# lixinghe1999/VRVQ

Hardware: AMD Instinct MI355X
Metric: audio-sec/s encode+RVQ+decode, 44.1 kHz batch-32, 1->8 MI355X; RVQ HBM GB/s (higher is better)
Workload: dtype f32; 1 GPU; DAC_VRVQ VBR 8 cb, level 1.0, 1-s clips, preprocess+encode+decode (z_q_is materialised); model=DAC_VRVQ base (8 cb), global_batch=32, clip_samples=44100, n_codebooks=8, parallelism=dp1 (replicas, no data-path collective)

## Files before the change

### include/vrvq.h

```cpp
#ifndef VRVQ_H_
#define VRVQ_H_

#include <stdint.h>

#ifdef __cplusplus
extern "C" {
#endif

typedef void* vrvq_stream_t;

enum vrvq_status_t {
  VRVQ_OK = 0,
  VRVQ_ERR_ARG = 10001,
  VRVQ_ERR_UNSUPPORTED = 10002
};

enum vrvq_epilogue_t { VRVQ_EPI_NONE = 0, VRVQ_EPI_TANH = 1, VRVQ_EPI_SIGMOID = 2 };

const char* vrvq_status_string(int status);
int vrvq_version(void);


int vrvq_weight_norm(const float* g, const float* v, int rows, int cols, float* w,
                     vrvq_stream_t stream);

int vrvq_snake_inv_alpha(const float* alpha, int channels, float* inv, vrvq_stream_t stream);

int vrvq_snake(const float* x, int batch, int channels, int frames, const float* alpha,
               const float* inv_alpha, float* y, vrvq_stream_t stream);

int vrvq_phase_split(const float* x, int batch, int channels, int frames, int stride, int pad,
                     int out_frames, const float* alpha, const float* inv_alpha, float* y,
                     vrvq_stream_t stream);

int vrvq_codebook_prep(const float* cb, int rows, int dim, float* cbn, float* c2,
                       vrvq_stream_t stream);

int vrvq_conv1d(const float* x, int batch, int cin, int tin, const float* alpha,
                const float* inv_alpha, const float* w_packed, const uint16_t* w_x3, int cout,
                int cout_pad, int k,
                int stride, int pad, int dil, const float* bias, const float* residual,
                int epilogue, float* y, int tout, const float* alpha_out,
                const float* inv_alpha_out, float* y_snake, vrvq_stream_t stream);

int vrvq_conv1d_workspace(int batch, int cin, int tin, int cout, int k, int stride, int pad,
                          int dil, int x3, long long* bytes);
int vrvq_conv1d_ws(const float* x, int batch, int cin, int tin, const float* alpha,
                   const float* inv_alpha, const float* w_packed, const uint16_t* w_x3, int cout,
                   int cout_pad, int k, int stride, int pad, int dil, const float* bias,
                   const float* residual, int epilogue, float* y, int tout,
                   const float* alpha_out, const float* inv_alpha_out, float* y_snake,
                   void* workspace, long long ws_bytes, vrvq_stream_t stream);

int vrvq_x3_weight_size(int cin, int k, int cout_pad, long long* n_u16);
int vrvq_pack_x3_weight(const float* w_packed, int cin, int k, int cout_pad, uint16_t* w_x3,
                        vrvq_stream_t stream);

int vrvq_conv1d_proj(const float* x, int batch, int cin, int tin, const float* alpha,
                     const float* inv_alpha, const float* w_packed, const uint16_t* w_x3, int cout,
                     int cout_pad, int k, int pad, int dil, const float* bias, float* y, int tout,
                     const uint16_t* w3in, int nq, float* part, void* workspace,
                     long long ws_bytes, vrvq_stream_t stream);

int vrvq_conv_last_launch(int out[5]);

enum vrvq_plan_kind_t { VRVQ_PLAN_CONV = 0, VRVQ_PLAN_PROJ = 1, VRVQ_PLAN_CONV_TRANSPOSE = 2 };
int vrvq_conv_plan(int kind, int batch, int cin, int tin, int cout, int k, int stride, int pad,
                   int dil, int has_x3, int has_workspace, int out[7]);

int vrvq_pack_conv1d_weight(const float* w, int cout, int cin, int k, int cout_pad,
                            float* w_packed, vrvq_stream_t stream);

int vrvq_residual_unit(const float* x, const float* x_snk, int batch, int channels, int frames,
                       int dil, const float* w7_packed, const uint16_t* w7_x3,
                       const uint16_t* w1_x3, const float* b7,
                       const float* alpha2,
                       const float* inv_alpha2, const float* w1_packed, const float* b1,
                       int cout_pad, float* y, const float* alpha_out,
                       const float* inv_alpha_out, float* y_snake, vrvq_stream_t stream);

int vrvq_conv_transpose1d(const float* x, int batch, int cin, int tin, const float* alpha,
                          const float* inv_alpha, const float* w_packed, int cout,
                          int cout_pad, int stride, const float* bias, float* y,
                          const float* alpha_out, const float* inv_alpha_out, float* y_snake,
                          vrvq_stream_t stream);

int vrvq_conv_transpose1d_pad(const float* x, int batch, int cin, int tin, const float* alpha,
                              const float* inv_alpha, const float* w_packed,
                              const uint16_t* w_x3, int cout,
                              int cout_pad, int stride, int pad, const float* bias, float* y,
                              const float* alpha_out, const float* inv_alpha_out,
                              float* y_snake, vrvq_stream_t stream);

int vrvq_pack_convt1d_weight(const float* w, int cin, int cout, int stride, int cout_pad,
                             float* w_packed, vrvq_stream_t stream);


int vrvq_rvq_cross_prep(const float* w_in_t, const float* w_out, const float* b_out, int nq,
                        int dim, int cdim, float* mcol, float* qb, vrvq_stream_t stream);

int vrvq_rvq_frag(const float* cbn, int nq, int ncode, int cdim, float* cbf,
                  vrvq_stream_t stream);

int vrvq_rvq_project_variant(int variant);

int vrvq_rvq_workspace(int batch, int frames, int nq, long long* bytes);

int vrvq_rvq_path(int path);

int vrvq_rvq_sync_error(vrvq_stream_t stream, int* code);
int vrvq_rvq_pending_error(int* code);
int vrvq_rvq_debug(unsigned spin_max, unsigned stall);

int vrvq_rvq_timing(int on);
int vrvq_rvq_timing_read(float* mean_ms, int* count);

int vrvq_rvq_w_in_planes_size(int nq, int dim, int cdim, long long* n_u16);
int vrvq_rvq_pack_w_in(const float* w_in_t, int nq, int dim, int cdim, uint16_t* w3in,
                       vrvq_stream_t stream);

int vrvq_rvq_workspace_part(int batch, int frames, int nq, int ncode, long long* bytes);
// ... 146 lines not shown
```

### vrvq_amd/_lib.py

```python
from __future__ import annotations

import ctypes
import os
import threading

LIB_NAME = "libvrvq_hip.so"
LIB_PATH = os.environ.get("VRVQ_LIB") or os.path.join(os.path.dirname(os.path.abspath(__file__)), LIB_NAME)

_P = ctypes.c_void_p
_I = ctypes.c_int
_F = ctypes.c_float

SIGNATURES = {
    "vrvq_weight_norm": [_P, _P, _I, _I, _P, _P],
    "vrvq_snake_inv_alpha": [_P, _I, _P, _P],
    "vrvq_snake": [_P, _I, _I, _I, _P, _P, _P, _P],
    "vrvq_phase_split": [_P, _I, _I, _I, _I, _I, _I, _P, _P, _P, _P],
    "vrvq_codebook_prep": [_P, _I, _I, _P, _P, _P],
    "vrvq_conv1d": [_P, _I, _I, _I, _P, _P, _P, _P, _I, _I, _I, _I, _I, _I, _P, _P, _I, _P, _I,
                    _P, _P, _P, _P],
    "vrvq_conv1d_workspace": [_I, _I, _I, _I, _I, _I, _I, _I, _I, _P],
    "vrvq_conv1d_ws": [_P, _I, _I, _I, _P, _P, _P, _P, _I, _I, _I, _I, _I, _I, _P, _P, _I, _P,
                       _I, _P, _P, _P, _P, ctypes.c_longlong, _P],
    "vrvq_conv1d_proj": [_P, _I, _I, _I, _P, _P, _P, _P, _I, _I, _I, _I, _I, _P, _P, _I, _P, _I,
# ... 16 lines not shown
    "vrvq_rvq_pack_w_in": [_P, _I, _I, _I, _P, _P],
    "vrvq_rvq_workspace_part": [_I, _I, _I, _I, _P],
    "vrvq_rvq_encode_part": [_P, _I, _I, _I, _I, _I, _I, _P, _P, _P, _P, _P, _P, _P, _P, _P, _F,
                             _P, _P, _P, _P, _P, _P, _P, ctypes.c_longlong, _P],
    "vrvq_rvq_fused_clips": [_I, _I, _I, _P],
    "vrvq_rvq_project": [_P, _I, _I, _I, _I, _I, _P, _P, _P],
    "vrvq_rvq_chain": [_P, _I, _I, _I, _I, _I, _P, _P, _P, _P, _P, _P, _P, _F, _P, _P, _P, _P, _P,
                       _P],
    "vrvq_rvq_expand": [_P, _I, _I, _I, _I, _I, _P, _P, _P, _F, _P, _P, _P, _P],
    "vrvq_rvq_gather": [_P, _I, _I, _I, _P, _I, _I, _P, _P, _P, _P],
    "vrvq_masked_loss": [_P, _P, _I, _I, _I, _P, _P],
    "vrvq_mask_hard": [_P, _I, _I, _I, _P, _P],
    "vrvq_scale_imp": [_P, _I, _F, _F, _P, _P],
    "vrvq_masked_sum": [_P, _P, _I, _I, _I, _I, _P, _P],
    "vrvq_bpf": [_P, _P, _I, _I, _I, _P, _P],
    "vrvq_rate_curve": [_P, _I, _I, _I, _P, _P, _I, _P, _P],
    "vrvq_rate_solve": [_P, _I, _I, _I, _P, _P, _I, _P, _F, _F, _P, _P, _P, _P],
    "vrvq_scale_imp_rows": [_P, _I, _I, _P, _P, _P],
    "vrvq_signal_metrics_workspace": [_I, ctypes.c_longlong, _P],
    "vrvq_signal_metrics": [_P, _P, _I, _I, ctypes.c_longlong, _P, _P, _P, _P, ctypes.c_longlong,
                            _P],
    "vrvq_spectral_distance_workspace": [_I, ctypes.c_longlong, _I, _P, _P],
    "vrvq_spectral_distance": [_P, _P, _I, _I, ctypes.c_longlong, _P, _I, _P, _P, _P, _P, _P,
                               ctypes.c_double, ctypes.c_double, ctypes.c_double, ctypes.c_double,
                               _P, _P, _P, ctypes.c_longlong, _P],
    "vrvq_pack_counts": [_P, _I, _I, _I, _P, _P, _P, _P, _P],
    "vrvq_pack_codes": [_P, _P, _P, _I, _I, _I, _I, _P, _P, _P],
    "vrvq_unpack_offsets": [_P, _I, _I, _P, _P, _P],
    "vrvq_unpack_codes": [_P, _P, _P, _I, _I, _I, _P, _P, _P],
    "vrvq_rvq_nearest": [_P, _I, _I, _I, _I, _P, _P, _I, _I, _P, _P],
    "vrvq_wgrad_plan": [_I, _I, _I, _I, _I, _P, _P],
    "vrvq_conv1d_wgrad": [_P, _I, _I, _I, _P, _P, _P, _I, _I, _P, _P, _I, _I, _I, _I, _I, _P,
                          ctypes.c_longlong, _P, _P],
    "vrvq_snake_backward_workspace": [_I, _I, _I, _P],
    "vrvq_snake_backward": [_P, _P, _P, _P, _I, _I, _I, _P, _P, _P, ctypes.c_longlong, _P],
    "vrvq_bias_grad_workspace": [_I, _I, _I, _P],
    "vrvq_bias_grad": [_P, _I, _I, _I, _P, _P, ctypes.c_longlong, _P],
    "vrvq_act_backward": [_P, _P, ctypes.c_longlong, _I, _P, _P],
    "vrvq_weight_norm_backward": [_P, _P, _P, _I, _I, _P, _P, _P],
    "vrvq_pack_conv1d_flip": [_P, _I, _I, _I, _I, _P, _P],
    "vrvq_mask_ste": [_P, _P, _P, _I, _I, _I, _F, _I, _I, _P, _P],
    "vrvq_mask_ste_backward": [_P, _P, _P, _I, _I, _I, _F, _I, _P, _P],
    "vrvq_rvq_expand_masked": [_P, _I, _I, _I, _I, _I, _P, _P, _P, _P, _P, _P],
    "vrvq_rvq_backward_workspace": [_I, _I, _I, _P],
    "vrvq_rvq_backward": [_P, _P, _P, _P, _P, _P, _P, _P, _I, _I, _I, _I, _I, _I, _P, _P, _P,
                          _P, _P, _P, _P, _P, _P, _P, _P, _P, _P, ctypes.c_longlong, _P],
}
EXTRA = {"vrvq_status_string": ([_I], ctypes.c_char_p), "vrvq_version": ([], _I),
         "vrvq_rvq_project_variant": ([_I], _I), "vrvq_rvq_path": ([_I], _I),
         "vrvq_rvq_sync_error": ([_P, _P], _I), "vrvq_rvq_timing": ([_I], _I),
         "vrvq_rvq_timing_read": ([_P, _P], _I), "vrvq_rvq_pending_error": ([_P], _I),
         "vrvq_rvq_debug": ([ctypes.c_uint, ctypes.c_uint], _I),
         "vrvq_rvq_debug_capacity": ([_I], _I), "vrvq_conv_last_launch": ([_P], _I),
         "vrvq_conv_plan": ([_I] * 11 + [_P], _I)}

METRICS_CHUNK = 16384
SPECTRAL_TILE_SAMPLES = 8192


def spectral_tile_frames(window: int) -> int:
    return SPECTRAL_TILE_SAMPLES // int(window)

_lock = threading.Lock()
_lib = None


def load() -> ctypes.CDLL:
    global _lib
    if _lib is not None:
        return _lib
    with _lock:
        if _lib is not None:
            return _lib
        if not os.path.exists(LIB_PATH):
            raise RuntimeError(
                f"vrvq_amd: HIP library {LIB_PATH} is missing; build it with "
                "`python -c 'import __graft_entry__ as g; g.build()'` (hipcc, gfx950)")
        lib = ctypes.CDLL(LIB_PATH)
        for name, argtypes in SIGNATURES.items():
            fn = getattr(lib, name)
            fn.argtypes = argtypes
            fn.restype = _I
        for name, (argtypes, restype) in EXTRA.items():
            fn = getattr(lib, name)
            fn.argtypes = argtypes
            fn.restype = restype
        _lib = lib
    return _lib


def call(name: str, *args) -> None:
    lib = load()
    rc = getattr(lib, name)(*args)
    if rc != 0:
        msg = lib.vrvq_status_string(rc)
        raise RuntimeError(f"{name} failed ({rc}): {msg.decode() if msg else 'unknown'}")


def rvq_path(path: int = 0) -> int:
    prev = load().vrvq_rvq_path(path)
    if prev not in (1, 2):
        raise RuntimeError(f"vrvq_rvq_path({path}) failed ({prev})")
    return prev


def rvq_sync_error(stream: int) -> int:
    code = ctypes.c_int(0)
    call("vrvq_rvq_sync_error", ctypes.c_void_p(stream), ctypes.byref(code))
    return code.value


def rvq_pending_error() -> int:
    code = ctypes.c_int(0)
    call("vrvq_rvq_pending_error", ctypes.byref(code))
    return code.value


def rvq_debug(spin_max: int = 0, stall: int = 0) -> None:
    call("vrvq_rvq_debug", ctypes.c_uint(spin_max), ctypes.c_uint(stall))


def rvq_fused_clips(frames: int, nq: int, ncode: int = 1024) -> int:
    n = ctypes.c_int(0)
    call("vrvq_rvq_fused_clips", frames, nq, ncode, ctypes.byref(n))
    return n.value


def rvq_debug_capacity(clips: int) -> int:
    return int(load().vrvq_rvq_debug_capacity(int(clips)))


def conv_last_launch() -> dict:
    out = (ctypes.c_int * 5)()
    call("vrvq_conv_last_launch", out)
    return dict(zip(("BM", "BN", "KS", "x3", "S"), (int(v) for v in out)))


PLAN_KINDS = {"conv": 0, "proj": 1, "convt": 2}


def conv_plan(kind, batch: int, cin: int, tin: int, cout: int, k: int, stride: int = 1,
              pad: int = 0, dil: int = 1, x3: bool = True, workspace: bool = True) -> dict:
    out = (ctypes.c_int * 7)()
    call("vrvq_conv_plan", PLAN_KINDS.get(kind, kind), batch, cin, tin, cout, k, stride, pad, dil,
         1 if x3 else 0, 1 if workspace else 0, out)
    return dict(zip(("BM", "BN", "KS", "x3", "S", "path", "WM"), (int(v) for v in out)))


def rvq_timing(on: bool) -> bool:
    return bool(load().vrvq_rvq_timing(1 if on else 0))


def rvq_timing_read():
    ms, n = ctypes.c_float(0.0), ctypes.c_int(0)
    call("vrvq_rvq_timing_read", ctypes.byref(ms), ctypes.byref(n))
    return float(ms.value), int(n.value)


def rvq_project_variant(variant: int = 0) -> int:
    prev = load().vrvq_rvq_project_variant(variant)
    if prev not in (1, 2, 3):
        raise RuntimeError(f"vrvq_rvq_project_variant({variant}) failed ({prev})")
    return prev
```

### vrvq_amd/csrc/conv.hip

```cpp
#include "common.h"
#include "conv_core.h"
#include "conv_x3.h"
#include <atomic>

namespace {

using namespace vrvq_conv;

template <int BM, int BN, int WM, int NW, int KS, bool X3, bool PH = false,
          bool PAIR = x3_pair<KS, BM, BN>(), bool SPLIT = false>
__global__ __launch_bounds__(64 * NW)
__attribute__((amdgpu_waves_per_eu(X3 && x3_stages<BM, BN>() == 1 ? 2 : 1)))
void conv_mfma_kernel(ConvArgs a) {
  using TC = TileCfg<BM, BN, WM, NW>;
  extern __shared__ __attribute__((aligned(16))) float smem[];
  int bid = blockIdx.x;
  int ks = 0;
  if (SPLIT) {
    ks = bid % a.ks_split;
    bid /= a.ks_split;
  }
  const int mt = bid % a.n_mt;
  bid /= a.n_mt;
  const int nt = bid % a.n_nt;
  const int b = bid / a.n_nt;
  const int m0 = mt * BM;
  const int n0 = nt * BN;
  f32x16 acc[TC::RM][TC::RN];
#pragma unroll
  for (int i = 0; i < TC::RM; ++i)
#pragma unroll
    for (int j = 0; j < TC::RN; ++j)
#pragma unroll
      for (int r = 0; r < 16; ++r) acc[i][j][r] = 0.0f;
  constexpr bool XPF = X3 && KS == 7 && PAIR && !SPLIT;
#ifdef VRVQ_X3_SB_ALL
  constexpr bool SB = true;
#else
  constexpr bool SB = KS == 1 || (KS == 2 && BN == 128) || XPF;
#endif
  if constexpr (X3) {
    if constexpr (SPLIT) {
      constexpr int CK = X3Cfg<KS, PAIR>::CK;
      const int nch = (a.cin + CK - 1) / CK, per = (nch + a.ks_split - 1) / a.ks_split;
      if (ks * per < nch)
        conv_mainloop_x3<BM, BN, WM, NW, KS, PH, PAIR, SB>(a, smem, acc, b, m0, n0, ks * per,
                                                            min(nch, (ks + 1) * per));
      constexpr int NR = TC::RM * TC::RN * 16;
      const size_t tile = ((size_t)b * a.n_nt + nt) * a.n_mt + mt;
      const size_t ntile = (size_t)gridDim.x / a.ks_split;
      float* dst = a.ks_part + ((size_t)ks * ntile + tile) * (size_t)NR * 64 * NW +
                   (threadIdx.x >> 6) * NR * 64 + (threadIdx.x & 63);
#pragma unroll
      for (int i = 0; i < TC::RM; ++i)
#pragma unroll
        for (int j = 0; j < TC::RN; ++j)
#pragma unroll
          for (int r = 0; r < 16; ++r) dst[((i * TC::RN + j) * 16 + r) * 64] = acc[i][j][r];
      return;
    }
    conv_mainloop_x3<BM, BN, WM, NW, KS, PH, PAIR, SB, XPF>(a, smem, acc, b, m0, n0);
  } else {
    conv_mainloop<BM, BN, WM, NW, KS>(a, smem, acc, b, m0, n0);
  }
  conv_epilogue<BM, BN, WM, NW>(a, smem, acc, b, m0, n0);
}

template <int BM, int BN, int WM, int NW>
__global__ __launch_bounds__(64 * NW) void conv_splitk_epilogue_kernel(ConvArgs a) {
  using TC = TileCfg<BM, BN, WM, NW>;
  extern __shared__ __attribute__((aligned(16))) float smem[];
  int bid = blockIdx.x;
  const int mt = bid % a.n_mt;
  bid /= a.n_mt;
  const int nt = bid % a.n_nt;
  const int b = bid / a.n_nt;
  constexpr int NR = TC::RM * TC::RN * 16;
  const size_t tile = blockIdx.x;
  const size_t pstride = (size_t)gridDim.x * NR * 64 * NW;
  const float* src = a.ks_part + tile * (size_t)NR * 64 * NW + (threadIdx.x >> 6) * NR * 64 +
                     (threadIdx.x & 63);
  f32x16 acc[TC::RM][TC::RN];
#pragma unroll
  for (int i = 0; i < TC::RM; ++i)
#pragma unroll
    for (int j = 0; j < TC::RN; ++j)
#pragma unroll
      for (int r = 0; r < 16; ++r) acc[i][j][r] = src[((i * TC::RN + j) * 16 + r) * 64];
  for (int s = 1; s < a.ks_split; ++s)
#pragma unroll
    for (int i = 0; i < TC::RM; ++i)
#pragma unroll
      for (int j = 0; j < TC::RN; ++j)
#pragma unroll
        for (int r = 0; r < 16; ++r)
          acc[i][j][r] = acc[i][j][r] + src[s * pstride + ((i * TC::RN + j) * 16 + r) * 64];
  conv_epilogue<BM, BN, WM, NW>(a, smem, acc, b, mt * BM, nt * BN);
}

constexpr int SMALL_BT = 256;
constexpr int SMALL_SC = 16;
constexpr int SMALL_COUT = 8;
constexpr int SMALL_WMAX = 2048;

template <int COUT>
__global__ __launch_bounds__(256) void conv_small_cout_kernel(ConvArgs a, int ks) {
  extern __shared__ __attribute__((aligned(16))) float sm[];
  float* w_s = sm;
  float* xs = sm + SMALL_WMAX;
  const int XW = SMALL_BT + (ks - 1) * a.dil;
  const int n_t = (a.ng + SMALL_BT - 1) / SMALL_BT;
  const int b = blockIdx.x / n_t;
  const int t0 = (blockIdx.x - b * n_t) * SMALL_BT;
  const int tid = threadIdx.x;
  const float* xb = a.x + (size_t)b * a.cin * a.tin;
  for (int e = tid; e < a.cin * ks * COUT; e += 256) {
    const int c = e % COUT, rk = e / COUT;
    w_s[e] = a.w[(size_t)rk * a.m_pad + c];
  }
  float acc[COUT];
#pragma unroll
  for (int c = 0; c < COUT; ++c) acc[c] = 0.0f;

  const int pmax = min(XW, a.ng - t0 + (ks - 1) * a.dil);
  for (int ci0 = 0; ci0 < a.cin; ci0 += SMALL_SC) {
    const int nc = min(SMALL_SC, a.cin - ci0);
    const int total = nc * pmax;
    for (int e0 = tid; e0 < total; e0 += 8 * 256) {
      float v[8];
#pragma unroll
      for (int u = 0; u < 8; ++u) {
// ... 163 lines not shown
    }
    const float bb = a.bias ? a.bias[co] : 0.0f;
    const size_t o = ((size_t)b * a.cout + co) * a.ylen + t0;
#pragma unroll
    for (int u = 0; u < CI1_T; ++u) v[u] = v[u] + bb;
    if (a.res) {
#pragma unroll
      for (int u = 0; u < CI1_T; ++u)
        if (full || t0 + u < a.ng) v[u] = a.res[o + u] + v[u];
    }
#pragma unroll
    for (int u = 0; u < CI1_T; ++u) v[u] = apply_epi(v[u], a.epi);
    if (a.y) {
      if (full) *reinterpret_cast<float4*>(a.y + o) = make_float4(v[0], v[1], v[2], v[3]);
      else
        for (int u = 0; u < CI1_T; ++u)
          if (t0 + u < a.ng) a.y[o + u] = v[u];
    }
    if (a.ys) {
      snake_n1<CI1_T>(v, a.alpha_o[co], a.inv_alpha_o[co]);
      if (full) *reinterpret_cast<float4*>(a.ys + o) = make_float4(v[0], v[1], v[2], v[3]);
      else
        for (int u = 0; u < CI1_T; ++u)
          if (t0 + u < a.ng) a.ys[o + u] = v[u];
    }
  }
}

enum ConvPath { PATH_MFMA = 0, PATH_SMALL_COUT = 1, PATH_CIN1 = 2 };
struct ConvPlan {
  int path;
  int BM, BN, WM;
  int KS;
  int x3;
  int S;
};

std::atomic<unsigned> g_last_launch{0};

void note_launch(const ConvPlan& p) {
  g_last_launch.store((unsigned)p.BM | (unsigned)p.BN << 9 | (unsigned)p.KS << 18 |
                      (unsigned)p.x3 << 23 | (unsigned)(p.S & 127) << 25,
                      std::memory_order_relaxed);
}

int finish(int rc, const ConvPlan& p, ConvPlan* plan) {
  if (rc == 0) {
    if (plan) *plan = p;
    else note_launch(p);
  }
  return rc;
}

int launch_kernel(void (*kernel)(ConvArgs), long long nblk, int threads, size_t lds,
                  hipStream_t st, const ConvArgs& a, bool dry) {
  if (dry) return 0;
  if (lds > 64 * 1024) {
    hipError_t e = hipFuncSetAttribute(reinterpret_cast<const void*>(kernel),
                                       hipFuncAttributeMaxDynamicSharedMemorySize, (int)lds);
    if (e != hipSuccess) return (int)e;
  }
  ConvArgs arg = a;
  void* params[] = {&arg};
  hipError_t e = hipLaunchKernel(reinterpret_cast<const void*>(kernel), dim3((unsigned)nblk),
                                 dim3(threads), params, lds, st);
  return e != hipSuccess ? (int)e : vrvq_launch_status();
}

int launch_small(const ConvArgs& a, int batch, int ks, hipStream_t st, ConvPlan* plan) {
  const ConvPlan p{PATH_SMALL_COUT, 0, 0, 0, ks, 0, 0};
  if (a.M == 1 && a.cout == 1 && a.stride == 1 && a.dil == 1 && a.tin % 4 == 0 &&
      ((ks == 7 && a.pad == 3) || (ks == 3 && a.pad == 1))) {
    const long long nblk = (long long)batch * ((a.ng + 256 * C1_T - 1) / (256 * C1_T));
    if (nblk <= 0 || nblk > 0x7fffffffLL) return VRVQ_ERR_ARG;
    if (plan) *plan = p;
    void (*kernel)(ConvArgs) =
        ks == 7 ? (a.alpha ? conv_cout1_stream_kernel<7, 3, true> : conv_cout1_stream_kernel<7, 3, false>)
                : (a.alpha ? conv_cout1_stream_kernel<3, 1, true> : conv_cout1_stream_kernel<3, 1, false>);
    return launch_kernel(kernel, nblk, 256, 0, st, a, plan != nullptr);
  }
  if (a.cin * ks * (a.M == 1 ? 1 : SMALL_COUT) > SMALL_WMAX) return VRVQ_ERR_UNSUPPORTED;
  const size_t lds = (size_t)(SMALL_WMAX + SMALL_SC * (SMALL_BT + (ks - 1) * a.dil)) * sizeof(float);
  if (lds > 64 * 1024) return VRVQ_ERR_UNSUPPORTED;
  const long long nblk = (long long)batch * ((a.ng + SMALL_BT - 1) / SMALL_BT);
  if (nblk <= 0 || nblk > 0x7fffffffLL) return VRVQ_ERR_ARG;
  if (plan) {
    *plan = p;
    return 0;
  }
  if (a.M == 1)
    hipLaunchKernelGGL(conv_small_cout_kernel<1>, dim3((unsigned)nblk), dim3(256), lds, st, a, ks);
  else
    hipLaunchKernelGGL(conv_small_cout_kernel<SMALL_COUT>, dim3((unsigned)nblk), dim3(256), lds, st, a, ks);
  return vrvq_launch_status();
}

template <int BM, int BN, int WM, int NW, int KS, bool PAIR, bool SPLIT = false>
int launch_x3(const ConvArgs& a, int XW, size_t epi, long long nblk, hipStream_t st, bool dry) {
  size_t lx = x3_lds_bytes<KS, BM, BN, PAIR>(XW, a.alpha ? (a.psh ? a.cin >> a.psh : a.cin) : 0);
  if (lx < epi) lx = epi;
  if (lx > 160 * 1024) return VRVQ_ERR_UNSUPPORTED;
  constexpr bool PH_TILE = KS == 2 && (x3_pair<KS, BM, BN>() || SPLIT);
  if constexpr (PH_TILE) {
    if (a.psh)
      return launch_kernel(conv_mfma_kernel<BM, BN, WM, NW, KS, true, true, PAIR, SPLIT>, nblk,
                           64 * NW, lx, st, a, dry);
  }
  if constexpr (SPLIT && KS == 2) {
    return VRVQ_ERR_ARG;
  } else {
    if (a.psh) return VRVQ_ERR_ARG;
    return launch_kernel(conv_mfma_kernel<BM, BN, WM, NW, KS, true, false, PAIR, SPLIT>, nblk,
                         64 * NW, lx, st, a, dry);
  }
}

template <int BM, int BN, int WM, int NW, int KS>
int launch_cfg(const ConvArgs& a0, int batch, hipStream_t st, ConvPlan* plan) {
  ConvArgs a = a0;
  a.n_mt = (a.M + BM - 1) / BM;
  a.n_nt = (a.ng + BN - 1) / BN;
  if (a.m_pad < a.n_mt * BM) return VRVQ_ERR_ARG;
  if (a.up > 0 && BM % a.up != 0) return VRVQ_ERR_UNSUPPORTED;
  constexpr int CK = ChunkCfg<KS, BM, BN>::CK;
  const int XW = (BN - 1) * a.stride + (KS - 1) * a.dil + 1;
  const int XP = a.ssh ? (XW + a.stride - 1) >> a.ssh : XW;
  const int XWP = a.ssh ? ((XP << a.ssh) + 3) & ~3 : (XW + 3) & ~3;
  size_t epi = (size_t)BM * EpiCfg<BM, BN, NW / WM>::BNP * sizeof(float);
  if (a.pj_part) {
    if (BM != 128) return VRVQ_ERR_UNSUPPORTED;
    if (epi < (size_t)PJE_LDS) epi = PJE_LDS;
  }
  const long long nblk = (long long)a.n_mt * a.n_nt * batch;
  if (nblk <= 0 || nblk > 0x7fffffffLL) return VRVQ_ERR_ARG;
  ConvPlan p{PATH_MFMA, BM, BN, WM, KS, 0, 0};
  const bool dry = plan != nullptr;
  if constexpr (NW == 4 && BM <= 192 && (KS == 1 || KS == 2 || KS == 3 || KS == 7)) {
    constexpr int XW_MAX = (BN - 1) + (KS - 1) * (KS == 7 ? 9 : 1) + 1;
    if (a.w3 != nullptr && a.stride == 1 && a.ssh == 0 && XW <= XW_MAX) {
      int rc;
      if (x3_pair<KS, BM, BN>() && a.cin % X3Cfg<KS, true>::CK == 0) {
        p.x3 = 2;
        rc = launch_x3<BM, BN, WM, NW, KS, x3_pair<KS, BM, BN>()>(a, XW, epi, nblk, st, dry);
      } else {
        p.x3 = 1;
        rc = launch_x3<BM, BN, WM, NW, KS, false>(a, XW, epi, nblk, st, dry);
      }
      if (rc != VRVQ_ERR_UNSUPPORTED) return finish(rc, p, plan);
      p.x3 = 0;
    }
  }
  if (a.psh) return VRVQ_ERR_UNSUPPORTED;
  if (XW > 64 * WinCfg<KS, BN>::PER_ROW) return VRVQ_ERR_UNSUPPORTED;
  size_t lds = 2 * (size_t)(CK * KS * BM + CK * XWP) * sizeof(float);
  if (lds < epi) lds = epi;
  if (lds > 160 * 1024) return VRVQ_ERR_UNSUPPORTED;
  return finish(launch_kernel(conv_mfma_kernel<BM, BN, WM, NW, KS, false>, nblk, 64 * NW, lds, st,
                              a, dry), p, plan);
}

constexpr int SPLITK_PARTS = 4;
constexpr int SPLITK_MIN_CHUNKS = 8;

int splitk_parts(int M, int cin, int ng, int ks, bool psh, bool up, bool x3) {
  if (!x3 || up || ng > 96 || M % 128 != 0) return 0;
  if (!(ks == 3 || ks == 7 || (ks == 2 && psh))) return 0;
  const int ck = ks == 2 ? X3Cfg<2, true>::CK : ks == 3 ? X3Cfg<3>::CK : X3Cfg<7>::CK;
  if (ks == 2 && cin % ck != 0) return 0;
  const int nch = (cin + ck - 1) / ck;
  const int S = nch / SPLITK_MIN_CHUNKS < SPLITK_PARTS ? nch / SPLITK_MIN_CHUNKS : SPLITK_PARTS;
  return S >= 2 ? S : 0;
}

size_t splitk_bytes(int S, int M, int ng, int batch) {
  return S ? (size_t)S * batch * (M / 128) * ((ng + 95) / 96) * 128 * 96 * sizeof(float) : 0;
}

template <int KS>
int launch_splitk(const ConvArgs& a0, int batch, int S, hipStream_t st, ConvPlan* plan) {
  if constexpr (KS == 2 || KS == 3 || KS == 7) {
    ConvArgs a = a0;
    a.ks_split = S;
    a.n_mt = a.M / 128;
    a.n_nt = (a.ng + 95) / 96;
    if (a.m_pad < a.n_mt * 128) return VRVQ_ERR_ARG;
    const int XW = 95 + (KS - 1) * a.dil + 1;
    constexpr int XW_MAX = 95 + (KS - 1) * (KS == 7 ? 9 : 1) + 1;
    if (XW > XW_MAX) return VRVQ_ERR_UNSUPPORTED;
    size_t epi = (size_t)128 * EpiCfg<128, 96, 1>::BNP * sizeof(float);
    if (a.pj_part && epi < (size_t)PJE_LDS) epi = PJE_LDS;
    const long long tiles = (long long)a.n_mt * a.n_nt * batch;
    if (tiles * S > 0x7fffffffLL) return VRVQ_ERR_ARG;
    const ConvPlan p{PATH_MFMA, 128, 96, 4, KS, KS == 2 ? 2 : 1, S};
    const bool dry = plan != nullptr;
    int rc = launch_x3<128, 96, 4, 4, KS, KS == 2, true>(a, XW, epi, tiles * S, st, dry);
    if (rc == 0)
      rc = launch_kernel(conv_splitk_epilogue_kernel<128, 96, 4, 4>, tiles, 256, epi, st, a, dry);
    return finish(rc, p, plan);
  } else {
    (void)a0; (void)batch; (void)S; (void)st; (void)plan;
    return VRVQ_ERR_UNSUPPORTED;
  }
}

constexpr long long BN96_MIN_WORKGROUPS = 384;

template <int KS>
int tile_width(const ConvArgs& a, int batch) {
  const bool x3_2tap = KS == 2 && a.w3 != nullptr;
  if (a.ng <= 32) return 32;
  if (a.ng <= 96) {
    if (x3_2tap) return a.up > 0 ? 96 : 32;
    return (long long)((a.M + 127) / 128) * batch >= BN96_MIN_WORKGROUPS ? 96 : 32;
  }
  auto waste = [&](int bn) { return ((a.ng + bn - 1) / bn) * bn - a.ng; };
  if (a.ng < 4096 && KS != 16 && waste(64) * 10 < waste(128) * 7 &&
      !(x3_2tap && (a.psh > 0 || a.up > 0)))
    return 64;
  return 128;
}

constexpr int K7_PAIR_MIN_COLUMNS = 640;

template <int BM, int WM, int KS>
int launch_bn(int bn, const ConvArgs& a, int batch, hipStream_t st, ConvPlan* plan) {
  if constexpr (KS != 16) {
    if (bn == 64) return launch_cfg<BM, 64, WM, 4, KS>(a, batch, st, plan);
  }
  return launch_cfg<BM, 128, WM, 4, KS>(a, batch, st, plan);
}

template <int KS>
int dispatch_tiles(const ConvArgs& a, int batch, hipStream_t st, ConvPlan* plan) {
  if (a.ks_part != nullptr) {
    const int S = splitk_parts(a.M, a.cin, a.ng, KS, a.psh > 0, a.up > 0, a.w3 != nullptr);
    if (S > 0) {
      const int rc = launch_splitk<KS>(a, batch, S, st, plan);
      if (rc != VRVQ_ERR_UNSUPPORTED) return rc;
    }
  }
  const int bn = tile_width<KS>(a, batch);
  const bool x3 = a.w3 != nullptr;
  if constexpr (KS == 2) {
    if (a.up > 0 && 128 % a.up != 0) return launch_bn<192, 2, KS>(bn <= 96 ? 64 : bn, a, batch, st, plan);
  }
  if (a.M <= 32) return launch_cfg<32, 128, 1, 4, KS>(a, batch, st, plan);
// ... 124 lines not shown
  const long long n = x3_size_u16(cin, k, cout_pad);
  if (n < 0) return VRVQ_ERR_UNSUPPORTED;
  const size_t total = (size_t)n / 8;
  const unsigned grid = (unsigned)((total + 255) / 256 < 65536 ? (total + 255) / 256 : 65536);
  u32x4* out = reinterpret_cast<u32x4*>(w_x3);
  hipStream_t st = as_stream(stream);
  switch (k) {
    case 1: hipLaunchKernelGGL(pack_x3_kernel<1>, dim3(grid), dim3(256), 0, st, w_packed, cin, cout_pad, out, total); break;
    case 2: hipLaunchKernelGGL(pack_x3_kernel<2>, dim3(grid), dim3(256), 0, st, w_packed, cin, cout_pad, out, total); break;
    case 3: hipLaunchKernelGGL(pack_x3_kernel<3>, dim3(grid), dim3(256), 0, st, w_packed, cin, cout_pad, out, total); break;
    default: hipLaunchKernelGGL(pack_x3_kernel<7>, dim3(grid), dim3(256), 0, st, w_packed, cin, cout_pad, out, total); break;
  }
  return vrvq_launch_status();
}

extern "C" int vrvq_conv1d(const float* x, int batch, int cin, int tin, const float* alpha,
                           const float* inv_alpha, const float* w_packed,
                           const uint16_t* w_x3, int cout,
                           int cout_pad, int k, int stride, int pad, int dil, const float* bias,
                           const float* residual, int epilogue, float* y, int tout,
                           const float* alpha_out, const float* inv_alpha_out, float* y_snake,
                           vrvq_stream_t stream) {
  return vrvq_conv1d_ws(x, batch, cin, tin, alpha, inv_alpha, w_packed, w_x3, cout, cout_pad, k,
                        stride, pad, dil, bias, residual, epilogue, y, tout, alpha_out,
                        inv_alpha_out, y_snake, nullptr, 0, stream);
}

extern "C" int vrvq_conv1d_workspace(int batch, int cin, int tin, int cout, int k, int stride,
                                     int pad, int dil, int x3, long long* bytes) {
  VRVQ_CHECK_ARG(bytes && batch > 0 && cin > 0 && tin > 0 && cout > 0 && k > 0 && stride > 0 &&
                 dil > 0 && pad >= 0);
  const long long tout = ((long long)tin + 2LL * pad - (long long)dil * (k - 1) - 1) / stride + 1;
  VRVQ_CHECK_ARG(tout > 0);
  int S = 0;
  if (stride > 1) {
    if (x3 && k == 2 * stride && (stride & (stride - 1)) == 0 && pad < stride)
      S = splitk_parts(cout, cin * stride, (int)tout, 2, true, false, true);
  } else {
    S = splitk_parts(cout, cin, (int)tout, k, false, false, x3 != 0);
  }
  *bytes = (long long)splitk_bytes(S, cout, (int)tout, batch);
  return 0;
}

extern "C" int vrvq_conv_last_launch(int out[5]) {
  VRVQ_CHECK_ARG(out);
  const unsigned v = g_last_launch.load(std::memory_order_relaxed);
  out[0] = (int)(v & 511);
  out[1] = (int)(v >> 9 & 511);
  out[2] = (int)(v >> 18 & 31);
  out[3] = (int)(v >> 23 & 3);
  out[4] = (int)(v >> 25 & 127);
  return 0;
}

namespace {


bool conv1d_geometry_ok(int batch, int cin, int tin, int cout, int cout_pad, int k, int stride,
                        int pad, int dil, int tout) {
  return batch > 0 && cin > 0 && tin > 0 && cout > 0 && k > 0 && stride > 0 && dil > 0 &&
         pad >= 0 && tout > 0 && cout_pad >= cout && cout_pad % 128 == 0 &&
         tout == ((long long)tin + 2LL * pad - (long long)dil * (k - 1) - 1) / stride + 1;
}

int run_conv1d(ConvArgs a, int batch, int cin, int tin, int cout, int cout_pad, int k, int stride,
               int pad, int dil, int tout, int epilogue, void* workspace, long long ws_bytes,
               hipStream_t st, ConvPlan* plan) {
  const bool proj = a.pj_part != nullptr;
  a.cin = cin; a.tin = tin; a.M = cout; a.m_pad = cout_pad; a.cout = cout;
  a.stride = stride; a.pad = pad; a.dil = dil; a.ng = tout; a.up = 0; a.up_pad = 0;
  a.ssh = 0;
  if (stride > 1 && (stride & (stride - 1)) == 0)
    while ((1 << a.ssh) < stride) ++a.ssh;
  a.ylen = tout; a.epi = epilogue;
  if (workspace != nullptr) {
    long long need = 0;
    const int rc = vrvq_conv1d_workspace(batch, cin, tin, cout, k, stride, pad, dil,
                                         a.w3 != nullptr, &need);
    if (rc) return rc;
    VRVQ_CHECK_ARG(ws_bytes >= need);
    if (need > 0) a.ks_part = static_cast<float*>(workspace);
  }
  if (a.w3 != nullptr && stride > 1) {
    if (k != 2 * stride || a.ssh == 0 || pad >= stride) return VRVQ_ERR_UNSUPPORTED;
    a.psh = a.ssh; a.ppad = pad; a.pcin = cin; a.ptin = tin;
    a.cin = cin * stride; a.tin = tout + 1;
    a.stride = 1; a.pad = 0; a.dil = 1; a.ssh = 0;
    return dispatch_ks(2, a, batch, st, plan);
  }
  if (!proj && cout <= SMALL_COUT && stride == 1 &&
      cin * k * (cout == 1 ? 1 : SMALL_COUT) <= SMALL_WMAX)
    return launch_small(a, batch, k, st, plan);
  if (!proj && cin == 1 && k == 7 && stride == 1 && dil == 1 && !a.alpha && cout % CI1_CG == 0 &&
      tout % 4 == 0) {
    const long long nblk =
        (long long)batch * ((tout + 256 * CI1_T - 1) / (256 * CI1_T)) * (cout / CI1_CG);
    if (nblk <= 0 || nblk > 0x7fffffffLL) return VRVQ_ERR_ARG;
    if (plan) *plan = ConvPlan{PATH_CIN1, 0, 0, 0, k, 0, 0};
    return launch_kernel(conv_cin1_stream_kernel<7>, nblk, 256, 0, st, a, plan != nullptr);
  }
  return dispatch_ks(k, a, batch, st, plan);
}

int run_conv_transpose1d(ConvArgs a, int batch, int cin, int tin, int cout, int cout_pad,
                         int stride, int pad, hipStream_t st, ConvPlan* plan) {
// ... 146 lines not shown
```

### vrvq_amd/csrc/conv_core.h

```cpp
#pragma once
#include "common.h"
#include <type_traits>

typedef float f32x16 __attribute__((ext_vector_type(16)));

namespace vrvq_conv {

struct ConvArgs {
  const float* x;
  const float* alpha;
  const float* inv_alpha;
  const float* w;
  const float* bias;
  const float* res;
  float* y;
  const float* alpha_o;
  const float* inv_alpha_o;
  float* ys;
  int cin, tin;
  int M;
  int m_pad;
  int cout;
  int stride, pad, dil;
  int ssh;
  int ng;
  int up, up_pad;
  int ylen;
  int epi;
  int n_mt, n_nt;
  const unsigned* w3;
  int psh, ppad, pcin, ptin;
  const unsigned* pj_w3;
  float* pj_part;
  int pj_nq;
  int pj_nf;
  int ks_split;
  float* ks_part;
};

__device__ __forceinline__ void split3x2_core(float v0, float v1, unsigned& h, unsigned& m,
                                              unsigned& l) {
  typedef __bf16 bf16x2_ __attribute__((ext_vector_type(2)));
  typedef float f32x2_ __attribute__((ext_vector_type(2)));
  const f32x2_ v = {v0, v1};
  const unsigned hu = __builtin_bit_cast(unsigned, __builtin_convertvector(v, bf16x2_));
  const f32x2_ hf = {__uint_as_float(hu << 16), __uint_as_float(hu & 0xffff0000u)};
  const f32x2_ r = v - hf;
  const unsigned mu = __builtin_bit_cast(unsigned, __builtin_convertvector(r, bf16x2_));
  const f32x2_ mf = {__uint_as_float(mu << 16), __uint_as_float(mu & 0xffff0000u)};
  const f32x2_ s = r - mf;
  h = hu;
  m = mu;
  l = __builtin_bit_cast(unsigned, __builtin_convertvector(s, bf16x2_));
}

template <int KS, int BM, int BN>
struct ChunkCfg {
  static constexpr int CK0 = KS == 1 ? 32 : KS <= 3 ? 16 : KS == 4 ? 8 : KS == 7 ? 8
                             : KS == 8 ? 4 : BN > 32 ? 4 : 2;
  static constexpr int CK = (BM > 128 && CK0 >= 8) ? CK0 / 2 : CK0;
};

__device__ __forceinline__ float apply_epi(float v, int epi) {
  if (epi == VRVQ_EPI_TANH) return tanhf(v);
  if (epi == VRVQ_EPI_SIGMOID) return 1.0f / (1.0f + expf(-v));
  return v;
}

template <int KS, int BN>
struct WinCfg {
  static constexpr int SMAX = (KS == 4 || KS == 8 || KS == 16) ? KS / 2 : 1;
  static constexpr int DMAX = KS == 7 ? 9 : 1;
  static constexpr int XW_MAX = (BN - 1) * SMAX + (KS - 1) * DMAX + 1;
  static constexpr int PER_ROW = (XW_MAX + 63) / 64;
};

template <int BM, int BN, int WN>
struct EpiCfg {
  static constexpr int need = (BM * BN * 4 + 65535) / 65536;
  static constexpr int EPASS = need <= 1 ? 1 : need <= 2 ? 2 : need <= 4 ? 4 : 8;
  static_assert(WN % EPASS == 0 || EPASS == 1, "epilogue passes must split the wave columns");
  static constexpr int BNP = BN / EPASS;
};


template <int BM, int BN, int WM, int NW>
struct TileCfg {
  static constexpr int NT = 64 * NW;
  static constexpr int WN = NW / WM;
  static constexpr int TM = BM / WM;
// ... 428 lines not shown
```

### vrvq_amd/csrc/misc.hip

```cpp
#include "common.h"

namespace {

__global__ __launch_bounds__(256) void weight_norm_kernel(const float* __restrict__ g,
                                                          const float* __restrict__ v, int cols,
                                                          float* __restrict__ w) {
  __shared__ float part[256];
  const size_t row = blockIdx.x;
  const float* vr = v + row * cols;
  float ss = 0.0f;
  for (int c = threadIdx.x; c < cols; c += 256) ss = fmaf(vr[c], vr[c], ss);
  part[threadIdx.x] = ss;
  __syncthreads();
  for (int h = 128; h >= 1; h >>= 1) {
    if ((int)threadIdx.x < h) part[threadIdx.x] += part[threadIdx.x + h];
    __syncthreads();
  }
  const float scale = g[row] / sqrtf(part[0]);
  for (int c = threadIdx.x; c < cols; c += 256) w[row * cols + c] = vr[c] * scale;
}

__global__ void inv_alpha_kernel(const float* __restrict__ alpha, int n, float* __restrict__ inv) {
  const int i = blockIdx.x * blockDim.x + threadIdx.x;
  if (i < n) inv[i] = 1.0f / (alpha[i] + 1e-9f);
// ... 163 lines not shown
  float e[8];
#pragma unroll
  for (int k = 0; k < 8; ++k) {
    e[k] = z[k] / nrm;
    q[k] = e[k] * e[k];
  }
  const float e2 = ((q[0] + q[1]) + (q[2] + q[3])) + ((q[4] + q[5]) + (q[6] + q[7]));
  float best = INFINITY;
  int bi = 0;
  for (int c = 0; c < ncode; ++c) {
    const float* r = cb_s + c * 8;
    float d = r[0] * e[0];
#pragma unroll
    for (int k = 1; k < 8; ++k) d = fmaf(r[k], e[k], d);
    const float dist = fmaf(d, -2.0f, e2) + c2_s[c];
    if (dist < best) {
      best = dist;
      bi = c;
    }
  }
  codes[((size_t)b * nq + i) * frames + t] = bi;
}

}

extern "C" int vrvq_rvq_nearest(const float* latents, int batch, int nlat, int frames, int nq,
                                const float* cbn, const float* c2, int ncode, int cdim,
                                int64_t* codes, vrvq_stream_t stream) {
  VRVQ_CHECK_ARG(latents && cbn && c2 && codes && batch > 0 && frames > 0 && nq > 0);
  VRVQ_CHECK_ARG(ncode > 0 && nlat >= nq * 8);
  if (cdim != 8 || ncode > 4096) return VRVQ_ERR_UNSUPPORTED;
  const long long nf = (long long)batch * frames;
  VRVQ_CHECK_ARG((nf + 255) / 256 < 0x7fffffffLL);
  const size_t lds = (size_t)ncode * 9 * sizeof(float);
  if (lds > 64 * 1024) {
    hipError_t e = hipFuncSetAttribute((const void*)rvq_nearest_kernel,
                                       hipFuncAttributeMaxDynamicSharedMemorySize, (int)lds);
    if (e != hipSuccess) return (int)e;
  }
  hipLaunchKernelGGL(rvq_nearest_kernel, dim3((unsigned)((nf + 255) / 256), nq), dim3(256), lds,
                     as_stream(stream), latents, batch, nlat, frames, cbn, c2, ncode, codes, nq);
  return vrvq_launch_status();
}

extern "C" const char* vrvq_status_string(int status) {
  switch (status) {
    case VRVQ_OK: return "ok";
    case VRVQ_ERR_ARG: return "vrvq: invalid argument (null pointer, size or shape mismatch)";
    case VRVQ_ERR_UNSUPPORTED: return "vrvq: shape outside the instantiated kernel set";
    default: return hipGetErrorString((hipError_t)status);
  }
}

extern "C" int vrvq_version(void) { return 104; }

extern "C" int vrvq_weight_norm(const float* g, const float* v, int rows, int cols, float* w,
                                vrvq_stream_t stream) {
  VRVQ_CHECK_ARG(g && v && w && rows > 0 && cols > 0);
  hipLaunchKernelGGL(weight_norm_kernel, dim3(rows), dim3(256), 0, as_stream(stream), g, v, cols, w);
  return vrvq_launch_status();
}

__global__ __launch_bounds__(256) void snake_rows_kernel(const float* __restrict__ x,
                                                         const float* __restrict__ alpha,
                                                         const float* __restrict__ inv_alpha,
                                                         int channels, int frames, int nseg,
                                                         float* __restrict__ y) {
  const int row = blockIdx.x / nseg, seg = blockIdx.x - row * nseg;
  const int c = row % channels;
  const float al = alpha[c], ia = inv_alpha[c];
  const size_t base = (size_t)row * frames;
#pragma unroll
  for (int u = 0; u < 4; ++u) {
    const int t = seg * 1024 + u * 256 + (int)threadIdx.x;
    if (t < frames) y[base + t] = snake_act(x[base + t], al, ia);
  }
}

extern "C" int vrvq_snake(const float* x, int batch, int channels, int frames, const float* alpha,
                          const float* inv_alpha, float* y, vrvq_stream_t stream) {
  VRVQ_CHECK_ARG(x && alpha && inv_alpha && y && x != y && batch > 0 && channels > 0 && frames > 0);
  const int nseg = (frames + 1023) / 1024;
  const long long nblk = (long long)batch * channels * nseg;
  if (nblk > 0x7fffffffLL) return VRVQ_ERR_ARG;
  hipLaunchKernelGGL(snake_rows_kernel, dim3((unsigned)nblk), dim3(256), 0, as_stream(stream), x,
                     alpha, inv_alpha, channels, frames, nseg, y);
  return vrvq_launch_status();
}

__global__ __launch_bounds__(256) void phase_split_kernel(const float* __restrict__ x,
                                                          const float* __restrict__ alpha,
                                                          const float* __restrict__ inv_alpha,
                                                          int channels, int frames, int sh,
                                                          int pad, int out_frames,
                                                          float* __restrict__ y, long long n) {
  const long long e = (long long)blockIdx.x * 256 + threadIdx.x;
  if (e >= n) return;
  const int m = (int)(e % out_frames);
  const long long rowv = e / out_frames;
  const int vr = (int)(rowv % ((long long)channels << sh));
  const long long b = rowv / ((long long)channels << sh);
  const int c = vr >> sh, r = vr & ((1 << sh) - 1);
  const int t = (m << sh) + r - pad;
  float v = 0.0f;
  if (t >= 0 && t < frames) {
    v = x[(b * channels + c) * (long long)frames + t];
    if (alpha) v = snake_act(v, alpha[c], inv_alpha[c]);
// ... 88 lines not shown
```

Before: 763.5 audio-sec/s.

## Remap conv tile block order to group weight-tile reuse per XCD L2

```diff
diff --git a/include/vrvq.h b/include/vrvq.h
--- a/include/vrvq.h
+++ b/include/vrvq.h
@@ -67,6 +67,16 @@
 enum vrvq_plan_kind_t { VRVQ_PLAN_CONV = 0, VRVQ_PLAN_PROJ = 1, VRVQ_PLAN_CONV_TRANSPOSE = 2 };
 int vrvq_conv_plan(int kind, int batch, int cin, int tin, int cout, int k, int stride, int pad,
                    int dil, int has_x3, int has_workspace, int out[7]);
+
+enum vrvq_tile_order_t {
+  VRVQ_TILE_IDENTITY = 0,
+  VRVQ_TILE_GROUP_X = 1,
+  VRVQ_TILE_PIN_M = 2
+};
+
+int vrvq_conv_tile_map(int total, int G, int n_mt, int order, int p, int* logical);
+
+int vrvq_conv_force_tile_order(int order_or_minus1);
 
 int vrvq_pack_conv1d_weight(const float* w, int cout, int cin, int k, int cout_pad,
                             float* w_packed, vrvq_stream_t stream);
diff --git a/vrvq_amd/_lib.py b/vrvq_amd/_lib.py
--- a/vrvq_amd/_lib.py
+++ b/vrvq_amd/_lib.py
@@ -92,7 +92,9 @@
          "vrvq_rvq_timing_read": ([_P, _P], _I), "vrvq_rvq_pending_error": ([_P], _I),
          "vrvq_rvq_debug": ([ctypes.c_uint, ctypes.c_uint], _I),
          "vrvq_rvq_debug_capacity": ([_I], _I), "vrvq_conv_last_launch": ([_P], _I),
-         "vrvq_conv_plan": ([_I] * 11 + [_P], _I)}
+         "vrvq_conv_plan": ([_I] * 11 + [_P], _I),
+         "vrvq_conv_tile_map": ([_I] * 5 + [_P], _I),
+         "vrvq_conv_force_tile_order": ([_I], _I)}
 
 METRICS_CHUNK = 16384
 SPECTRAL_TILE_SAMPLES = 8192
@@ -187,6 +189,22 @@
     return dict(zip(("BM", "BN", "KS", "x3", "S", "path", "WM"), (int(v) for v in out)))
 
 
+TILE_ORDERS = {"identity": 0, "group_x": 1, "pin_m": 2}
+
+
+def conv_tile_map(total: int, G: int, n_mt: int, order, p: int) -> tuple:
+    out = (ctypes.c_int * 4)()
+    call("vrvq_conv_tile_map", total, G, n_mt, TILE_ORDERS.get(order, order), p, out)
+    return tuple(int(v) for v in out)
+
+
+def conv_force_tile_order(order=-1) -> int:
+    prev = load().vrvq_conv_force_tile_order(-1 if order is None else TILE_ORDERS.get(order, order))
+    if not -1 <= prev <= 2:
+        raise RuntimeError(f"vrvq_conv_force_tile_order({order}) failed ({prev})")
+    return prev
+
+
 def rvq_timing(on: bool) -> bool:
     return bool(load().vrvq_rvq_timing(1 if on else 0))
 
diff --git a/vrvq_amd/csrc/conv.hip b/vrvq_amd/csrc/conv.hip
--- a/vrvq_amd/csrc/conv.hip
+++ b/vrvq_amd/csrc/conv.hip
@@ -1,6 +1,7 @@
 #include "common.h"
 #include "conv_core.h"
 #include "conv_x3.h"
+#include "tile_order.h"
 #include <atomic>
 
 namespace {
@@ -14,7 +15,8 @@
 void conv_mfma_kernel(ConvArgs a) {
   using TC = TileCfg<BM, BN, WM, NW>;
   extern __shared__ __attribute__((aligned(16))) float smem[];
-  int bid = blockIdx.x;
+  int bid = tile_order_map(a.order, (int)gridDim.x, a.n_mt * (SPLIT ? a.ks_split : 1), a.n_mt,
+                           (int)blockIdx.x);
   int ks = 0;
   if (SPLIT) {
     ks = bid % a.ks_split;
@@ -70,13 +72,13 @@
 __global__ __launch_bounds__(64 * NW) void conv_splitk_epilogue_kernel(ConvArgs a) {
   using TC = TileCfg<BM, BN, WM, NW>;
   extern __shared__ __attribute__((aligned(16))) float smem[];
-  int bid = blockIdx.x;
+  const size_t tile = tile_order_map(a.order, (int)gridDim.x, a.n_mt, a.n_mt, (int)blockIdx.x);
+  int bid = (int)tile;
   const int mt = bid % a.n_mt;
   bid /= a.n_mt;
   const int nt = bid % a.n_nt;
   const int b = bid / a.n_nt;
   constexpr int NR = TC::RM * TC::RN * 16;
-  const size_t tile = blockIdx.x;
   const size_t pstride = (size_t)gridDim.x * NR * 64 * NW;
   const float* src = a.ks_part + tile * (size_t)NR * 64 * NW + (threadIdx.x >> 6) * NR * 64 +
                      (threadIdx.x & 63);
@@ -346,6 +348,33 @@
   return rc;
 }
 
+constexpr long long XCD_L2_BYTES = 4ll << 20;
+struct OrderRule {
+  int BM, BN, KS;
+  int n_mt_lo, n_mt_hi;
+  int w_fits;
+  int order;
+};
+constexpr OrderRule ORDER_RULES[] = {
+    {64, 256, 7, 8, 8, 0, TILE_GROUP_X},
+    {128, 64, 1, 4, 4, 1, TILE_GROUP_X},
+};
+
+std::atomic<int> g_force_order{-1};
+
+int tile_order_for(const ConvPlan& p, const ConvArgs& a) {
+  const int f = g_force_order.load(std::memory_order_relaxed);
+  if (f >= 0) return f;
+  if (a.n_mt < 2) return TILE_IDENTITY;
+  const long long wb = (long long)a.cin * p.KS * a.m_pad * (p.x3 ? 6 : 4);
+  const int fits = wb <= XCD_L2_BYTES;
+  for (const OrderRule& r : ORDER_RULES)
+    if (r.BM == p.BM && r.BN == p.BN && r.KS == p.KS && a.n_mt >= r.n_mt_lo &&
+        a.n_mt <= r.n_mt_hi && (r.w_fits < 0 || r.w_fits == fits))
+      return r.order;
+  return TILE_IDENTITY;
+}
+
 int launch_kernel(void (*kernel)(ConvArgs), long long nblk, int threads, size_t lds,
                   hipStream_t st, const ConvArgs& a, bool dry) {
   if (dry) return 0;
@@ -435,15 +464,18 @@
       int rc;
       if (x3_pair<KS, BM, BN>() && a.cin % X3Cfg<KS, true>::CK == 0) {
         p.x3 = 2;
+        a.order = tile_order_for(p, a);
         rc = launch_x3<BM, BN, WM, NW, KS, x3_pair<KS, BM, BN>()>(a, XW, epi, nblk, st, dry);
       } else {
         p.x3 = 1;
+        a.order = tile_order_for(p, a);
         rc = launch_x3<BM, BN, WM, NW, KS, false>(a, XW, epi, nblk, st, dry);
       }
       if (rc != VRVQ_ERR_UNSUPPORTED) return finish(rc, p, plan);
       p.x3 = 0;
     }
   }
+  a.order = tile_order_for(p, a);
   if (a.psh) return VRVQ_ERR_UNSUPPORTED;
   if (XW > 64 * WinCfg<KS, BN>::PER_ROW) return VRVQ_ERR_UNSUPPORTED;
   size_t lds = 2 * (size_t)(CK * KS * BM + CK * XWP) * sizeof(float);
@@ -486,6 +518,7 @@
     const long long tiles = (long long)a.n_mt * a.n_nt * batch;
     if (tiles * S > 0x7fffffffLL) return VRVQ_ERR_ARG;
     const ConvPlan p{PATH_MFMA, 128, 96, 4, KS, KS == 2 ? 2 : 1, S};
+    a.order = tile_order_for(p, a);
     const bool dry = plan != nullptr;
     int rc = launch_x3<128, 96, 4, 4, KS, KS == 2, true>(a, XW, epi, tiles * S, st, dry);
     if (rc == 0)
@@ -716,6 +749,22 @@
   out[3] = (int)(v >> 23 & 3);
   out[4] = (int)(v >> 25 & 127);
   return 0;
+}
+
+extern "C" int vrvq_conv_tile_map(int total, int G, int n_mt, int order, int p, int* logical) {
+  VRVQ_CHECK_ARG(logical && total > 0 && G > 0 && n_mt > 0 && G % n_mt == 0 && p >= 0 &&
+                 p < total && order >= 0 && order < TILE_ORDERS);
+  const int L = tile_order_map(order, total, G, n_mt, p), ksp = G / n_mt;
+  logical[0] = L;
+  logical[1] = L / G;
+  logical[2] = L / ksp % n_mt;
+  logical[3] = L % ksp;
+  return 0;
+}
+
+extern "C" int vrvq_conv_force_tile_order(int order_or_minus1) {
+  if (order_or_minus1 < -1 || order_or_minus1 >= TILE_ORDERS) return VRVQ_ERR_ARG;
+  return g_force_order.exchange(order_or_minus1, std::memory_order_relaxed);
 }
 
 namespace {
diff --git a/vrvq_amd/csrc/conv_core.h b/vrvq_amd/csrc/conv_core.h
--- a/vrvq_amd/csrc/conv_core.h
+++ b/vrvq_amd/csrc/conv_core.h
@@ -36,6 +36,7 @@
   int pj_nf;
   int ks_split;
   float* ks_part;
+  int order;
 };
 
 __device__ __forceinline__ void split3x2_core(float v0, float v1, unsigned& h, unsigned& m,
diff --git a/vrvq_amd/csrc/misc.hip b/vrvq_amd/csrc/misc.hip
--- a/vrvq_amd/csrc/misc.hip
+++ b/vrvq_amd/csrc/misc.hip
@@ -239,7 +239,7 @@
   }
 }
 
-extern "C" int vrvq_version(void) { return 104; }
+extern "C" int vrvq_version(void) { return 105; }
 
 extern "C" int vrvq_weight_norm(const float* g, const float* v, int rows, int cols, float* w,
                                 vrvq_stream_t stream) {
diff --git a/vrvq_amd/csrc/tile_order.h b/vrvq_amd/csrc/tile_order.h
--- /dev/null
+++ b/vrvq_amd/csrc/tile_order.h
@@ -0,0 +1,38 @@
+#pragma once
+
+#if defined(__HIPCC__) || defined(__CUDACC__)
+#define VRVQ_HD __host__ __device__
+#else
+#define VRVQ_HD
+#endif
+
+namespace vrvq_conv {
+
+enum TileOrder { TILE_IDENTITY = 0, TILE_GROUP_X = 1, TILE_PIN_M = 2, TILE_ORDERS = 3 };
+
+constexpr int TILE_XCDS = 8;
+
+VRVQ_HD inline int tile_pin_classes(int n_mt) {
+  return n_mt % 8 == 0 ? 8 : n_mt % 4 == 0 ? 4 : n_mt % 2 == 0 ? 2 : 1;
+}
+
+VRVQ_HD inline int tile_order_map(int order, int total, int G, int n_mt, int p) {
+  if (order == TILE_IDENTITY || G <= 0 || n_mt <= 0 || G % n_mt != 0) return p;
+  if (total / TILE_XCDS < G) return p;
+  const int sbn = TILE_XCDS * G;
+  const int sb = p / sbn;
+  if (sb >= total / sbn) return p;
+  const int q = p - sb * sbn;
+  const int x = q % TILE_XCDS, slot = q / TILE_XCDS;
+  if (order == TILE_GROUP_X) return sb * sbn + x * G + slot;
+  if (order != TILE_PIN_M) return p;
+  const int ksp = G / n_mt;
+  const int np = tile_pin_classes(n_mt);
+  const int per = G / np;
+  const int win = (x / np) * np + slot / per;
+  const int s = slot - (slot / per) * per;
+  const int mt = x % np + (s / ksp) * np;
+  return sb * sbn + win * G + mt * ksp + s % ksp;
+}
+
+}
```

After: 769.1 audio-sec/s (median of 6 runs). No clear change (+0.7%).
